# jonasrothfuss/ProMP

Measured on AMD Instinct MI355X. Metric: env-steps/sec through GAE+inner+outer update, higher is better.
Workload: dtype f32

## Files before the change

### include/promp_hip.h

```cpp
#ifndef PROMP_HIP_H
#define PROMP_HIP_H

#include <stddef.h>
#include <stdint.h>

#ifdef __cplusplus
extern "C" {
#endif

typedef struct promp_ctx promp_ctx;

typedef struct promp_dims {
    int32_t n_tasks;
    int32_t n_tasks_global;
    int32_t obs_dim;
    int32_t act_dim;
    int32_t hidden1, hidden2;
    int32_t num_inner_steps;
    int32_t max_rows;
    int32_t max_paths;
    int32_t n_hidden;
    int32_t hidden3, hidden4;
    int32_t hidden_act;
} promp_dims;
// ... 40 lines not shown
int promp_stage_wait(promp_ctx* ctx);
void* promp_host_alloc(size_t bytes);
void promp_host_free(void* p);

int promp_process_samples(promp_ctx* ctx, int step, const promp_proc_opts* opts);

int promp_download_processed(promp_ctx* ctx, int step, float* returns, float* advantages, double* coeffs,
                             double* path_returns0, double* path_undiscounted, double* path_reward_sumsq);

int promp_download_raw(promp_ctx* ctx, int step, double* returns64, double* raw_advantages64);

int promp_set_coeffs(promp_ctx* ctx, int step, int baseline_kind, const double* coeffs);
int promp_predict_baseline(promp_ctx* ctx, int step, int baseline_kind, double* baselines_out);

int promp_set_advantages(promp_ctx* ctx, int step, const float* advantages);
int promp_set_dice_rewards(promp_ctx* ctx, int step, const float* rewards);

int promp_set_theta(promp_ctx* ctx, const float* theta);
int promp_get_theta(promp_ctx* ctx, float* theta);
int promp_set_step_sizes(promp_ctx* ctx, const float* step_sizes);
int promp_set_learn_std(promp_ctx* ctx, int learn_std);
int promp_set_min_std(promp_ctx* ctx, float min_std);
int promp_set_schedule(promp_ctx* ctx, int stage_overlap, int fuse_min_tasks);
int promp_set_primal_cache(promp_ctx* ctx, int on);
int promp_set_reuse_adapt(promp_ctx* ctx, int on);
long long promp_adapt_passes_skipped(promp_ctx* ctx);
long long promp_constraint_hvp_cached_passes(promp_ctx* ctx);
long long promp_state_version(promp_ctx* ctx);
int promp_set_adam_state(promp_ctx* ctx, const float* m, const float* v, int64_t t);
int promp_get_adam_state(promp_ctx* ctx, float* m, float* v, int64_t* t);
int promp_switch_to_pre_update(promp_ctx* ctx);
int promp_set_task_thetas(promp_ctx* ctx, const float* theta_tasks);
int promp_get_task_thetas(promp_ctx* ctx, float* theta_tasks);

int promp_inner_adapt(promp_ctx* ctx, int step, int inner_kind);

int promp_policy_forward(promp_ctx* ctx, const float* obs, int batch, float* mean_out);

int promp_begin_rollout(promp_ctx* ctx, int step, int envs_per_task, int path_length);
int promp_begin_collection(promp_ctx* ctx, int step, int envs_per_task, int max_steps);
int promp_end_collection(promp_ctx* ctx, int step, int n_paths, const int32_t* task_path_offsets, const int32_t* path_env,
                         const int32_t* path_start, const int32_t* path_len, const float* rewards);
int promp_policy_step(promp_ctx* ctx, int step, int t, const float* obs, uint64_t seed, int clip_infos, float* actions_out);
int promp_set_rewards(promp_ctx* ctx, int step, const float* rewards);
int promp_set_rewards_f64(promp_ctx* ctx, int step, const double* rewards);

// ... 51 lines not shown
```

### promp_amd/_lib.py

```python
import ctypes as C
import os

import weakref

import numpy as np

_HERE = os.path.dirname(os.path.abspath(__file__))
DEFAULT_LIBRARY = os.path.join(_HERE, 'libpromp_hip.so')

BASELINE_ZERO, BASELINE_LINEAR_FEATURE, BASELINE_LINEAR_TIME = 0, 1, 2
INNER_RATIO, INNER_LOGLIK, INNER_DICE = 0, 1, 2
OUTER_CLIP, OUTER_RATIO, OUTER_KL, OUTER_LOGLIK = 0, 1, 2, 3
LOSS_RATIO, LOSS_CLIP, LOSS_LOGLIK, LOSS_KL = 0, 1, 2, 3
KERNEL_FWD_BWD, KERNEL_HVP, KERNEL_GRAM, KERNEL_FWD, KERNEL_EXCHANGE = 0, 1, 2, 3, 4


class PrompError(RuntimeError):
    pass


class Dims(C.Structure):
    _fields_ = [('n_tasks', C.c_int32), ('n_tasks_global', C.c_int32), ('obs_dim', C.c_int32), ('act_dim', C.c_int32),
                ('hidden1', C.c_int32), ('hidden2', C.c_int32), ('num_inner_steps', C.c_int32),
                ('max_rows', C.c_int32), ('max_paths', C.c_int32),
# ... 24 lines not shown
    'promp_last_error': (C.c_char_p, []),
    'promp_abi_version': (C.c_int, []),
    'promp_param_count': (C.c_int, [C.POINTER(Dims)]),
    'promp_feature_dim': (C.c_int, [C.POINTER(Dims), C.c_int]),
    'promp_sync': (C.c_int, [_P]),
    'promp_upload_step': (C.c_int, [_P, C.c_int, C.c_int, _I, _I, _F, _F, _F, _F, _F, C.c_int]),
    'promp_process_samples': (C.c_int, [_P, C.c_int, C.POINTER(ProcOpts)]),
    'promp_download_processed': (C.c_int, [_P, C.c_int, _F, _F, _D, _D, _D, _D]),
    'promp_download_raw': (C.c_int, [_P, C.c_int, _D, _D]),
    'promp_set_coeffs': (C.c_int, [_P, C.c_int, C.c_int, _D]),
    'promp_predict_baseline': (C.c_int, [_P, C.c_int, C.c_int, _D]),
    'promp_set_advantages': (C.c_int, [_P, C.c_int, _F]),
    'promp_set_theta': (C.c_int, [_P, _F]),
    'promp_get_theta': (C.c_int, [_P, _F]),
    'promp_set_step_sizes': (C.c_int, [_P, _F]),
    'promp_set_learn_std': (C.c_int, [_P, C.c_int]),
    'promp_set_primal_cache': (C.c_int, [_P, C.c_int]),
    'promp_set_reuse_adapt': (C.c_int, [_P, C.c_int]),
    'promp_adapt_passes_skipped': (C.c_longlong, [_P]),
    'promp_constraint_hvp_cached_passes': (C.c_longlong, [_P]),
    'promp_state_version': (C.c_longlong, [_P]),
    'promp_set_min_std': (C.c_int, [_P, C.c_float]),
    'promp_set_schedule': (C.c_int, [_P, C.c_int, C.c_int]),
    'promp_set_rewards_f64': (C.c_int, [_P, C.c_int, _D]),
    'promp_stage_step': (C.c_int, [_P, C.c_int, C.c_int, _I, _I, _F, _F, _F, _F, _F, C.c_int]),
    'promp_commit_step': (C.c_int, [_P, C.c_int]),
    'promp_stage_wait': (C.c_int, [_P]),
    'promp_host_alloc': (C.c_void_p, [C.c_size_t]),
    'promp_host_free': (None, [C.c_void_p]),
    'promp_constraint_hvp': (C.c_int, [_P, C.c_int, _F, C.c_int, _F]),
    'promp_cg_solve': (C.c_int, [_P, C.c_int, _F, C.c_int, C.c_float, C.c_float, C.c_int, C.c_float, _F, C.POINTER(C.c_double)]),
    'promp_set_adam_state': (C.c_int, [_P, _F, _F, C.c_int64]),
    'promp_get_adam_state': (C.c_int, [_P, _F, _F, C.POINTER(C.c_int64)]),
    'promp_switch_to_pre_update': (C.c_int, [_P]),
    'promp_set_task_thetas': (C.c_int, [_P, _F]),
    'promp_get_task_thetas': (C.c_int, [_P, _F]),
    'promp_inner_adapt': (C.c_int, [_P, C.c_int, C.c_int]),
    'promp_policy_forward': (C.c_int, [_P, _F, C.c_int, _F]),
    'promp_rollout_point_env': (C.c_int, [_P, C.c_int, C.c_int, C.c_int, _D, _D, _F, C.POINTER(PointEnvOpts)]),
    'promp_begin_rollout': (C.c_int, [_P, C.c_int, C.c_int, C.c_int]),
    'promp_begin_collection': (C.c_int, [_P, C.c_int, C.c_int, C.c_int]),
    'promp_end_collection': (C.c_int, [_P, C.c_int, C.c_int, _P, _P, _P, _P, _F]),
    'promp_policy_step': (C.c_int, [_P, C.c_int, C.c_int, _F, C.c_uint64, C.c_int, _F]),
    'promp_set_rewards': (C.c_int, [_P, C.c_int, _F]),
    'promp_download_step': (C.c_int, [_P, C.c_int, _F, _F, _F, _F, _F]),
    'promp_meta_grad': (C.c_int, [_P, C.c_float, _F, C.c_int, C.c_int, _F, _F]),
# ... 590 lines not shown
                   old_mean=np.empty((R, A), np.float32), old_log_std=np.empty((ls_rows, A), np.float32))
        self._call('promp_download_step', int(step), _ptr(out['obs'], C.c_float), _ptr(out['act'], C.c_float),
                   _ptr(out['rew'], C.c_float), _ptr(out['old_mean'], C.c_float), _ptr(out['old_log_std'], C.c_float))
        return out

    def inner_adapt(self, step, inner_kind=INNER_RATIO):
        self._call('promp_inner_adapt', int(step), int(inner_kind))

    def meta_grad(self, clip_eps, inner_kl_coeff, inner_kind=INNER_RATIO, outer_kind=OUTER_CLIP):
        eta = _f32(inner_kl_coeff)
        assert eta.shape == (self.K,)
        grad, stats = np.empty(self.n_params, np.float32), np.empty(self.K + 2, np.float32)
        self._call('promp_meta_grad', float(clip_eps), _ptr(eta, C.c_float), int(inner_kind), int(outer_kind),
                   _ptr(grad, C.c_float), _ptr(stats, C.c_float))
        return grad, dict(loss=float(stats[0]), inner_kl=stats[1:1 + self.K].copy(), outer_kl=float(stats[1 + self.K]))

    def meta_eval(self, clip_eps, inner_kl_coeff, inner_kind=INNER_RATIO, outer_kind=OUTER_CLIP):
        r = self.optimize(0, 0.0, clip_eps, inner_kl_coeff, inner_kind, outer_kind)
        return dict(loss=r['loss_after'], inner_kl=r['inner_kl'], outer_kl=r['outer_kl'])

    def set_schedule(self, stage_overlap=-1, fuse_min_tasks=-1):
        self._call('promp_set_schedule', int(stage_overlap), int(fuse_min_tasks))

    def set_primal_cache(self, on=True):
        self._call('promp_set_primal_cache', -1 if on is None else int(bool(on)))

    def set_reuse_adapt(self, on=True):
        self._call('promp_set_reuse_adapt', int(bool(on)))

    def adapt_passes_skipped(self):
        return int(self.lib.cdll.promp_adapt_passes_skipped(self._h))

    def state_version(self):
        return int(self.lib.cdll.promp_state_version(self._h))

    def constraint_hvp_cached_passes(self):
        return int(self.lib.cdll.promp_constraint_hvp_cached_passes(self._h))

    def set_min_std(self, min_std):
        self._call('promp_set_min_std', float(min_std))

    def set_learn_std(self, on=True):
        self._call('promp_set_learn_std', int(bool(on)))

    def adam_step(self, lr):
        self._call('promp_adam_step', float(lr))
# ... 156 lines not shown
```

### promp_amd/csrc/promp_hip.hip

```cpp
#include "promp_kernels_chain.h"
#include "promp_kernels_pass.h"
#include "promp_kernels_policy.h"
#include "promp_kernels_policy_wide.h"
#include "promp_kernels_wide_bf16.h"
#include "promp_kernels_sample.h"
#include "promp_kernels_rollout.h"
#include "promp_kernels_generic.h"
#include "promp_kernels_generic_bf16.h"
#include "../../include/promp_hip.h"

#include <algorithm>
#include <cmath>
#include <cstdarg>
#include <cstdio>
#include <cstdlib>
#include <cstring>
#include <memory>
#include <string>
#include <vector>

#define PROMP_ARCH_NAME(prop) (prop).gcnArchName

namespace {

// ... 173 lines not shown
    bool tasks_shared = false;
    DevBuf<float> wbuf;
    DevBuf<float> partials, scal_inner, scal_outer, scal_tmp;
    DevBuf<float> red, grad_mean, stats;
    float eta_last[PROMP_ETA_MAX] = {};
    DevBuf<double> gram_partials, red64;
    DevBuf<char> rollout_buf;
    DevBuf<float> stage_rows;
    DevBuf<double> fit_scratch;
    size_t smem_fwd = 0, smem_hvp = 0;
    PassFamily family = PassFamily::Chain;
    int wb_cls = 0;
    size_t smem_wb_fwd = 0, smem_wb_bwd = 0, smem_wb_hvp = 0;
    DevBuf<unsigned> wb_planes, wb_vplanes;
    DevBuf<unsigned> wb_planes_meta;
    DevBuf<float> cg_buf;
    DevBuf<double> cg_scal;
    struct { bool valid = false; unsigned long long theta_version = 0, data_version = 0, sizes_version = 0; const void* step = nullptr; } wbp;
    DevBuf<unsigned> vdir_absmax;
    bool gramt_single = false;
    bool gram_untiled = false;
    int gramt_map_nblk = -1;
    GramtMap gramt_map;
    bool fit_one_launch = false;
    bool gen_bf16 = true;
    DevBuf<unsigned short> gb_wplanes, gb_vplanes;
    long long gb_plane_stride = 0;
    int gb_pf_off[GEN_MAX_LIN] = {}, gb_pb_off[GEN_MAX_LIN] = {};
    int n_lin = 0, g_maxw = 0;
    GenLin lin[GEN_MAX_LIN];
    DevBuf<float> g_act[GEN_MAX_LIN], g_ract[GEN_MAX_LIN], g_mu, g_rmu, g_dz[2], g_qz[2];
    DevBuf<unsigned long long> dbg;
    bool dbg_enabled = false;
    DevBuf<int> task_counters;
    DevBuf<int> split_events;
    ncclComm_t comm = nullptr;
    int rank = 0, nranks = 1;
    float min_log_std = -13.815510558f;
    bool learn_std = true;
    int fuse_min_tasks = 1 << 30;
    int stats_slot = 0;
    int primal_cache = -1;
    unsigned long long version_counter = 0, theta_version = 0, sizes_version = 0;
    unsigned long long cache_counter = 0;
    unsigned long long opt_theta_version = 0;
    struct { bool valid = false; unsigned long long theta_version = 0, data_version = 0, sizes_version = 0; int inner_kind = 0; bool cached = false; float min_log_std = 0.f; bool learn_std = true; } adapt0;
// ... 692 lines not shown
    }
    {
        const int lds = 160 * 1024;
#define PROMP_CHAIN_LDS(N1, N2, KS) if (allow_lds(lds, k_chain_hvp<N1, N2, KS, CHAIN_NW_HVP, false>, k_chain_hvp<N1, N2, KS, CHAIN_NW_HVP, true>)) return -2;
        PROMP_CHAIN_ALL(PROMP_CHAIN_LDS)
#undef PROMP_CHAIN_LDS
#define PROMP_PASS_LDS(N1, N2) \
    if (allow_lds(lds, k_pass<N1, N2, CHAIN_NW_HVP, true, true>, k_pass<N1, N2, CHAIN_NW_HVP, true, false>, k_pass<N1, N2, CHAIN_NW_HVP, false, false>)) return -2;
        PROMP_PASS_ALL(PROMP_PASS_LDS)
#undef PROMP_PASS_LDS
#define PROMP_WB_LDS(CLS, NKO, NXB) if (allow_lds(lds, k_wb_hvp<NKO, NXB>, k_wb_fwd_bwd<NKO, NXB, true>, k_wb_fwd_bwd<NKO, NXB, false>)) return -2;
        PROMP_WB_ALL(PROMP_WB_LDS)
#undef PROMP_WB_LDS
#define PROMP_WIDE_LDS(HH, NOB) if (allow_lds(lds, k_wide_fwd_bwd<HH, NOB, true>, k_wide_fwd_bwd<HH, NOB, false>, k_wide_hvp<HH, NOB>)) return -2;
        PROMP_WIDE_ALL(PROMP_WIDE_LDS)
#undef PROMP_WIDE_LDS
#define PROMP_GEN_LDS(NBW)                                                                                                   \
    if (allow_lds(lds, k_gen_linear<GEN_FWD, NBW>, k_gen_linear<GEN_FWD_T, NBW>, k_gen_linear<GEN_BWD, NBW>, k_gen_linear<GEN_BWD_T, NBW>, \
                  k_gen_wgrad<1, NBW>, k_gen_wgrad<2, NBW>, k_gb_linear<GEN_FWD, NBW>, k_gb_linear<GEN_FWD_T, NBW>,            \
                  k_gb_linear<GEN_BWD, NBW>, k_gb_linear<GEN_BWD_T, NBW>, k_gb_wgrad<1, NBW>, k_gb_wgrad<2, NBW>)) return -2;
        PROMP_GEN_LDS(1) PROMP_GEN_LDS(2) PROMP_GEN_LDS(3) PROMP_GEN_LDS(4)
#undef PROMP_GEN_LDS
        if (allow_lds((int)gen_loss_smem(GEN_MAX_A), k_gen_loss<true, true>, k_gen_loss<false, true>, k_gen_loss<false, false>)) return -2;
#define PROMP_GRAM_INST(NBLK) k_gram<NBLK>,
#define PROMP_FITWV_INST(DT) k_fit_wave<DT>,
        if (allow_lds(lds, PROMP_GRAM_ALL(PROMP_GRAM_INST) PROMP_FITWV_ALL(PROMP_FITWV_INST) k_fit, k_gram_wide, k_gram_tiled<GRAMT_TB, GRAMT_NWV, GRAMT_NLD>, k_fitw_panel<32>, k_fitw_panel<16>,
                      k_fitw_update<32>, k_fitw_update<16>, k_fitw_back<32>, k_fitw_back<16>, k_fit_wide<32>, k_fit_wide<16>)) return -2;
#undef PROMP_GRAM_INST
#undef PROMP_FITWV_INST
    }
    const size_t NP = c->NP, MNP = (size_t)M * NP;
    if (c->theta.alloc(NP) || c->step_sizes.alloc(NP)) return -2;
    if (c->adam_m.alloc(NP) || c->adam_v.alloc(NP)) return -2;
    if (c->theta_tasks.alloc(MNP) || c->chain.alloc((size_t)(K + 1) * MNP)) return -2;
    if (c->lam.alloc(MNP) || c->vbuf.alloc(MNP)) return -2;
    if (c->family == PassFamily::CoopSplit) {
        const size_t pw = (size_t)M * wb_planes_words(wb_nko(c->wb_cls));
        if (c->wb_planes.alloc(pw) || c->wb_vplanes.alloc(pw) || c->wb_planes_meta.alloc(pw)) return -2;
        if (c->vdir_absmax.alloc((size_t)M)) return -2;
    }
    if (c->partials.alloc((size_t)c->max_work * c->partial_stride)) return -2;
    if (c->scal_inner.alloc((size_t)K * M * 2) || c->scal_outer.alloc((size_t)M * 2)) return -2;
    if (c->scal_tmp.alloc((size_t)M * 2)) return -2;
    if (c->red.alloc(NP + K + 2) || c->grad_mean.alloc(NP)) return -2;
    if (c->stats.alloc((size_t)2 * (K + 2))) return -2;
    if (c->red64.alloc(64)) return -2;
    if (c->family == PassFamily::Layered) {
        const size_t R = (size_t)dims->max_rows;
        for (int l = 1; l < c->n_lin; ++l)
// ... 334 lines not shown
    if (o->baseline_kind == PROMP_BASELINE_LINEAR_FEATURE && c->d.obs_dim > PROMP_LINFEAT_MAX_O)
        return fail(-1, "LinearFeatureBaseline's fit is sized for obs_dim <= %d (%d here: %d feature columns); fit LinearTimeBaseline / no "
                    "baseline on the device, or hand advantages in through promp_set_advantages", PROMP_LINFEAT_MAX_O, c->d.obs_dim,
                    2 * c->d.obs_dim + 5);
    SampleArgs a = sample_args(c, S, o->baseline_kind);
    a.work = S.work[0];
    a.task_wg_offsets = S.task_wg_offsets[0];
    a.gamma = o->discount; a.lam = o->gae_lambda; a.reg = o->reg_coeff;
    a.normalize = o->normalize_adv; a.positive = o->positive_adv;
    a.ret64 = S.ret64; a.ret32 = S.ret32; a.adv32 = S.adv32;
    a.path_ret0 = S.path_ret0; a.path_undisc = S.path_undisc; a.path_rsq = S.path_rsq;
    S.feat_dim = a.D;
    const bool on_side = c->overlap && !c->prof && step >= 1;
    hipStream_t st = on_side ? c->side : c->stream;
    if (o->baseline_kind != PROMP_BASELINE_ZERO && fit_buffers(c, on_side)) return -2;
    a.gram_partials = on_side ? c->gram_partials_side : c->gram_partials;
    double* fit_scratch = on_side ? c->fit_scratch_side : c->fit_scratch;
    if (on_side) {
        if (mark_use(c, S)) return -2;
        if (S.use_set) HIPCHECK(hipStreamWaitEvent(c->side, S.ev_use, 0));
        if (S.wait_ready_side) HIPCHECK(hipStreamWaitEvent(c->side, S.ev_ready, 0));
    }
    S.wait_ready_side = false;
    PROMP_LAUNCH(k_returns, dim3(S.n_paths), 64, 0, st, a);
    HIPCHECK(hipGetLastError());
    if (a.kind != BASE_ZERO) {
        const int nblk = (a.D + 1 + 15) / 16;
        if (prof_begin(c, PROMP_KERNEL_GRAM, S.n_rows)) return -2;
        const bool small = nblk <= 5 && (a.O <= 32 || a.kind != BASE_LINFEAT);
        switch (small ? nblk : 0) {
#define PROMP_GRAM_CASE(NBLK) \
    case NBLK: { auto k = k_gram<NBLK>; PROMP_LAUNCH(k, dim3(S.n_work[0]), 64 * GramCfg<NBLK>::NW, GramCfg<NBLK>::SMEM_BYTES, st, a); } break;
            PROMP_GRAM_ALL(PROMP_GRAM_CASE)
#undef PROMP_GRAM_CASE
            default:
                if (nblk >= GRAMT_MIN_NBLK && !c->gram_untiled) {
                    const int nr = gramt_nrect(nblk);
                    int rows, db;
                    gramt_cfg(nblk, a.O, 64 * GRAMT_NWV * GRAMT_NLD, c->gramt_single, &rows, &db);
                    if (c->gramt_map_nblk != nblk) { gramt_balance(nblk, GRAMT_NWV, &c->gramt_map); c->gramt_map_nblk = nblk; }
                    auto k = k_gram_tiled<GRAMT_TB, GRAMT_NWV, GRAMT_NLD>;
                    PROMP_LAUNCH(k, dim3(S.n_work[0], (nr + GRAMT_NWV - 1) / GRAMT_NWV), 64 * GRAMT_NWV, gramt_smem(nblk, rows, db), st, a, nblk,
                                 c->gramt_map, rows, db);
                    break;
                }
                PROMP_LAUNCH(k_gram_wide, dim3(S.n_work[0], gramw_slices(nblk)), 512, gramw_smem(nblk, a.O, gramw_rows(nblk, a.O)), st, a, nblk,
                             gramw_rows(nblk, a.O));
        }
        HIPCHECK(hipGetLastError());
        if (prof_end(c, PROMP_KERNEL_GRAM)) return -2;
        const int DA = a.D + 1;
        if (small) {
            const size_t fit_smem = sizeof(double) * ((size_t)2 * DA * DA + 3 * DA + 2 + fitwv_aux(64));
#define PROMP_FITWV_CASE(DT) else if (DA <= DT) { auto k = k_fit_wave<DT>; PROMP_LAUNCH(k, dim3(c->d.n_tasks), FITWV_NT, fit_smem, st, a, nblk); }
            if (false) {}
            PROMP_FITWV_ALL(PROMP_FITWV_CASE)
            else PROMP_LAUNCH(k_fit, dim3(c->d.n_tasks), 256, fit_smem, st, a, nblk);
#undef PROMP_FITWV_CASE
        } else {
            PROMP_LAUNCH(k_gram_sum_wide, dim3(c->d.n_tasks * fitw_sum_split(nblk)), 256, 0, st, a, nblk, fit_scratch, fitw_sum_split(nblk));
            HIPCHECK(hipGetLastError());
            const int* none = nullptr;
            int* bad = (int*)(fit_scratch + (size_t)c->d.n_tasks * 2 * (c->Dmax + 1) * (c->Dmax + 1));
            const bool phases = a.D >= FITW_ML_MIN_D && !c->fit_one_launch;
#define PROMP_FITW(NB)                                                                                                              \
    if (phases) {                                                                                                                   \
        auto kp = k_fitw_panel<NB>; auto ku = k_fitw_update<NB>; auto kb = k_fitw_back<NB>; auto kf = k_fit_wide<NB>;              \
        for (int k0 = 0; k0 < a.D; k0 += NB) {                                                                                      \
            PROMP_LAUNCH(kp, dim3(c->d.n_tasks), FITW_NT, fitw_panel_smem(a.D, NB), st, a, fit_scratch, k0);                        \
            if (k0 + NB < a.D) PROMP_LAUNCH(ku, dim3(c->d.n_tasks, FITW_UPD_SPLIT), FITW_NT, fitw_panel_smem(a.D, NB), st, a, fit_scratch, k0); \
        }                                                                                                                           \
        PROMP_LAUNCH(kb, dim3(c->d.n_tasks), FITW_NT, fitw_back_smem(a.D, NB), st, a, fit_scratch, bad);                               \
        PROMP_LAUNCH(kf, dim3(c->d.n_tasks), FITW_NT, fitw_smem(a.D, NB), st, a, nblk, fit_scratch, (const int*)bad);               \
    } else { auto k = k_fit_wide<NB>; PROMP_LAUNCH(k, dim3(c->d.n_tasks), FITW_NT, fitw_smem(a.D, NB), st, a, nblk, fit_scratch, none); }
            if (fitw_nb(a.D) == 32) { PROMP_FITW(32) } else { PROMP_FITW(16) }
#undef PROMP_FITW
        }
        HIPCHECK(hipGetLastError());
    }
    PROMP_LAUNCH(k_gae, dim3(S.n_paths), 64, sizeof(double) * (size_t)(a.D > 0 ? a.D : 1), st, a);
    HIPCHECK(hipGetLastError());
    a.work = S.work[1];
    PROMP_LAUNCH(k_normalize, dim3(S.n_work[1]), 256, 0, st, a);
    HIPCHECK(hipGetLastError());
    if (on_side) {
        HIPCHECK(hipEventRecord(S.ev_done, c->side));
        S.side_pending = true;
    }
    S.processed = true;
    S.has_adv = true;
    return 0;
}

int promp_download_processed(promp_ctx* c, int step, float* returns, float* adv, double* coeffs, double* ret0,
                             double* undisc, double* rsq) {
    StepScope sc(c, step, false, false);
    if (sc.rc) return sc.rc;
    StepData& S = sc.S();
    if (!S.processed) return fail(-3, "step %d has not been processed", step);
    hipStream_t st = c->stream;
    if (returns) HIPCHECK(hipMemcpyAsync(returns, S.ret32, sizeof(float) * S.n_rows, hipMemcpyDeviceToHost, st));
    if (adv) HIPCHECK(hipMemcpyAsync(adv, S.adv32, sizeof(float) * S.n_rows, hipMemcpyDeviceToHost, st));
    const size_t P = (size_t)S.n_paths, NC = (coeffs && S.feat_dim > 0) ? (size_t)c->d.n_tasks * c->coeff_stride : 0;
    if (c->small_host.reserve(3 * P + NC, 1)) return -2;
    double* h = c->small_host;
    if (ret0) HIPCHECK(hipMemcpyAsync(h, S.path_ret0, sizeof(double) * P, hipMemcpyDeviceToHost, st));
    if (undisc) HIPCHECK(hipMemcpyAsync(h + P, S.path_undisc, sizeof(double) * P, hipMemcpyDeviceToHost, st));
// ... 137 lines not shown
}
int promp_set_step_sizes(promp_ctx* c, const float* s) {
    NEED_CTX(c);
    c->sizes_version = ++c->version_counter;
    if (params_in(c, c->step_sizes, s, 1)) return -2;
    return mask_log_std_step_sizes(c);
}
int promp_set_min_std(promp_ctx* c, float min_std) {
    NEED_CTX(c);
    if (!(min_std > 0.f)) return fail(-1, "min_std must be positive");
    c->min_log_std = logf(min_std);
    c->version_counter += 1;
    return 0;
}
int promp_set_schedule(promp_ctx* c, int stage_overlap, int fuse_min_tasks) {
    NEED_CTX(c);
    if (stage_overlap >= 0) {
        HIPCHECK(hipStreamSynchronize(c->side));
        c->overlap = stage_overlap != 0;
    }
    if (fuse_min_tasks >= 0) c->fuse_min_tasks = fuse_min_tasks;
    return 0;
}
int promp_set_reuse_adapt(promp_ctx* c, int on) {
    NEED_CTX(c);
    c->reuse_adapt = on != 0;
    c->adapt0.valid = false;
    return 0;
}
long long promp_adapt_passes_skipped(promp_ctx* c) { return c ? c->adapt_passes_skipped : -1; }
long long promp_constraint_hvp_cached_passes(promp_ctx* c) { return c ? c->chvp_cached_passes : -1; }
long long promp_state_version(promp_ctx* c) { return c ? (long long)c->version_counter : -1; }
int promp_set_primal_cache(promp_ctx* c, int on) {
    NEED_CTX(c);
    c->primal_cache = on < 0 ? -1 : on != 0;
    return 0;
}
int promp_set_learn_std(promp_ctx* c, int on) {
    NEED_CTX(c);
    if (on && !c->learn_std) return fail(-3, "learn_std cannot be switched back on: the log_std step sizes were zeroed (set the step sizes again)");
    c->learn_std = on != 0;
    c->sizes_version = ++c->version_counter;
    return mask_log_std_step_sizes(c);
}
static int tasks_materialize(promp_ctx* c);
int promp_set_task_thetas(promp_ctx* c, const float* t) {
// ... 755 lines not shown
```

### promp_amd/csrc/promp_kernels_sample.h

```cpp
#pragma once
#include <utility>
#include "promp_device.h"
#include "promp_kernels_policy.h"

enum { BASE_ZERO = 0, BASE_LINFEAT = 1, BASE_LINTIME = 2 };

struct SampleArgs {
    const float* obs;
    const float* rew;
    const double* rew64;
    const int* path_row_offsets;
    const int* path_task;
    const int* row_t;
    const int* task_row_offsets;
    const int* task_path_offsets;
    const WorkItem* work;
    const int* task_wg_offsets;
    int O, D, kind;
    double gamma, lam, reg;
    int normalize, positive;
    double* ret64;
    float* ret32;
    double* adv64;
    float* adv32;
// ... 70 lines not shown
        for (int end = T; end > 0; end -= 64) {
            const int t = end - 64 + lane;
            const double x = (t >= 0) ? (double)a.c[row0 + t] : 0.0;
            const double y = dice_suffix_chunk(x, lane) + carry;
            if (t >= 0) a.tmp[row0 + t] = y;
            carry = shfl_idx_f64(y, 0);
        }
        total = carry;
    }
    double carry = 0.0;
    for (int end = T; end > 0; end -= 64) {
        const int t = end - 64 + lane;
        double x = 0.0;
        if (t >= 0) {
            x = (double)a.rw[row0 + t];
            if (a.mode == 1) x *= total - a.tmp[row0 + t] + (double)a.c[row0 + t];
        }
        const double y = dice_suffix_chunk(x, lane) + carry;
        if (t >= 0) a.out[row0 + t] = (float)y;
        carry = shfl_idx_f64(y, 0);
    }
}

template <int NBLK>
struct GramCfg {
    static constexpr int NW = (NBLK <= 3) ? 8 : 4;
    static constexpr int FS = (NBLK % 2 == 1) ? 16 * NBLK : 16 * NBLK + 16;
    static constexpr int NPAIR = NBLK * (NBLK + 1) / 2;
    static constexpr int WAVE_BYTES = 16 * FS * 8 + 16 * 32 * 4 + 2 * 16 * 8;
    static constexpr int SLAB_BYTES = NW * NPAIR * 256 * 8;
    static constexpr int SMEM_BYTES = (NW * WAVE_BYTES > SLAB_BYTES) ? NW * WAVE_BYTES : SLAB_BYTES;
};

#ifdef PROMP_DEV_STAMPS
#define SA_STAMPS unsigned long long ph[8] = {0, 0, 0, 0, 0, 0, 0, 0}, tph = promp_clock()
#define SA_PHASE(i) do { const unsigned long long now_ = promp_clock(); ph[i] += now_ - tph; tph = now_; } while (0)
#else
#define SA_STAMPS do { } while (0)
#define SA_PHASE(i) do { } while (0)
#endif
template <int NBLK>
__global__ void __launch_bounds__(64 * GramCfg<NBLK>::NW) k_gram(SampleArgs a) {
    SA_STAMPS;
    constexpr int NW = GramCfg<NBLK>::NW, FS = GramCfg<NBLK>::FS, NPAIR = GramCfg<NBLK>::NPAIR, NC = 16 * NBLK;
    PROMP_SMEM_DECL;
    unsigned char* smem = (unsigned char*)PROMP_SMEM_PTR;
    const int tid = threadIdx.x, lane = tid & 63, w = tid >> 6, i16 = lane & 15, kk = lane >> 4;
    double* Phi = (double*)(smem + (size_t)w * GramCfg<NBLK>::WAVE_BYTES);
    const WorkItem wk = a.work[blockIdx.x];
    const int O = a.O, D = a.D;
    f64x4 acc[NPAIR];
#pragma unroll
    for (int p = 0; p < NPAIR; ++p) acc[p] = zero4d();
    float xr[8];
    double tr = 0.0;
    int ttr = 0;
    auto request = [&](int base) {
        const bool live = base < wk.row_end;
        const int nrows = !live ? 0 : (wk.row_end - base) < 16 ? (wk.row_end - base) : 16;
        const long long b0 = live ? base : wk.row_begin;
        if (a.kind == BASE_LINFEAT) {
            const int lim = nrows * O;
#pragma unroll
            for (int u = 0; u < 8; ++u) {
                const int e = lane + 64 * u;
                const float x = a.obs[b0 * O + (e < lim ? e : 0)];
                xr[u] = (e < lim) ? x : 0.f;
            }
        }
        if (lane < 16) {
            const int r = lane < nrows ? lane : 0;
            tr = a.ret64[b0 + r];
            ttr = a.row_t[b0 + r];
        }
    };
    int poff[8];
#pragma unroll
    for (int u = 0; u < 8; ++u) {
        const int e = lane + 64 * u, r = e / (O > 0 ? O : 1);
        poff[u] = (a.kind == BASE_LINFEAT && e < 16 * O) ? r * FS + (e - r * O) : -1;
    }
    for (int e = lane; e < 16 * FS; e += 64) Phi[e] = 0.0;
    wave_sync();
    const int qt = (a.kind == BASE_LINFEAT) ? 2 * O : 0;
    request(wk.row_begin + 16 * w);
    SA_PHASE(0);
    for (int base = wk.row_begin + 16 * w; base < wk.row_end; base += 16 * NW) {
        const int nrows = (wk.row_end - base) < 16 ? (wk.row_end - base) : 16;
#pragma unroll
        for (int u = 0; u < 8; ++u)
            if (poff[u] >= 0) {
                const float oc = fminf(fmaxf(xr[u], -10.f), 10.f);
                Phi[poff[u]] = (double)oc;
                Phi[poff[u] + O] = (double)(oc * oc);
            }
        if (lane < 16) {
            const bool rv = lane < nrows;
            const double tau = rv ? (double)ttr / 100.0 : 0.0;
            double* pr = Phi + lane * FS;
            pr[qt] = tau;
            pr[qt + 1] = tau * tau;
            pr[qt + 2] = tau * tau * tau;
            pr[qt + 3] = rv ? 1.0 : 0.0;
            pr[D] = rv ? tr : 0.0;
        }
        SA_PHASE(1);
// ... 131 lines not shown
        const int k0 = J + 2 + 8 * b;
        double m[8];
        sched_fence();
#pragma unroll
        for (int u = 0; u < 8; ++u) m[u] = (k0 + u < DT) ? readlane_f64(W[J], k0 + u) : 0.0;
#pragma unroll
        for (int u = 0; u < 8; ++u)
            if (k0 + u < DT) W[k0 + u] -= W[J] * m[u];
        sched_fence();
        if (b == 0) e = rsq_e(dn, r0);
        if (b == 1 || (b == 0 && NBATCH == 1)) rs = rsq_finish(r0, e);
    }
    if (NBATCH <= 0) rs = rsq_finish(r0, rsq_e(dn, r0));
}
template <int DT, int... Js>
PROMP_DEV void fitw_columns(double (&W)[DT], double* colbuf, double* rsv, int lane, int D, std::integer_sequence<int, Js...>) {
    const double d0 = readlane_f64(W[0], 0), s0 = rsq_seed(d0);
    double rs = rsq_finish(s0, rsq_e(d0, s0));
    (fitw_column<Js, DT>(W, colbuf, rsv, rs, lane, D), ...);
}

#define FITWV_NT 512
template <int DT>
__global__ void __launch_bounds__(FITWV_NT) k_fit_wave(SampleArgs a, int NBLK) {
    PROMP_SMEM_DECL;
    SA_STAMPS;
    const int D = a.D, DA = D + 1;
    double* colbuf = (double*)PROMP_SMEM_PTR;
    double* rsv = colbuf + DT * FITWV_CS + 2;
    double* G = colbuf + fitwv_aux(DT);
    const int lane = threadIdx.x & 63, task = blockIdx.x;
    const int NPAIR = NBLK * (NBLK + 1) / 2;
    const int wg0 = a.task_wg_offsets[task], wg1 = a.task_wg_offsets[task + 1];
    {
        constexpr int NE = 5;
        double sacc[NE];
#pragma unroll
        for (int q = 0; q < NE; ++q) sacc[q] = 0.0;
        for (int base = wg0; base < wg1; base += 16) {
            double v[NE][16];
#pragma unroll
            for (int q = 0; q < NE; ++q) {
                const int e = threadIdx.x + q * FITWV_NT;
                if (e < NPAIR * 256) {
#pragma unroll
                    for (int u = 0; u < 16; ++u) {
                        const int wg = base + u < wg1 ? base + u : wg1 - 1;
                        v[q][u] = a.gram_partials[(long long)wg * (NPAIR * 256) + e];
                    }
                }
            }
#pragma unroll
            for (int q = 0; q < NE; ++q) {
                const int e = threadIdx.x + q * FITWV_NT;
// ... 35 lines not shown
        SA_PHASE(1);
        wave_fence();
        double y = (lane < D) ? colbuf[lane * FITWV_CS + D] : 0.0;
        const double rdg = rsv[lane < D ? lane : 0];
#pragma unroll
        for (int k = 0; k < DT; ++k) {
            const double l = colbuf[row * FITWV_CS + (k < DA ? k : 0)];
            W[k] = (k < D && row < k) ? l : 0.0;
        }
        SA_PHASE(2);
#pragma unroll
        for (int j = DT - 1; j >= 0; --j) {
            if (j < D) {
                const double wj = readlane_f64(y * rdg, j);
                y -= W[j] * wj;
            }
        }
        wsol = y * rdg;
        wave_sync();
        SA_PHASE(3);
        if (!wave_any(lane < D && wsol != wsol)) break;
        reg *= 10.0;
    }
    if (lane < D) a.coeffs[(long long)task * a.coeff_stride + lane] = wsol;
#ifdef PROMP_DEV_STAMPS
    if (task == 0 && lane == 0)
        printf("k_fit_wave cycles: partial sums %llu | factorisation %llu | column reads %llu | back substitution %llu\n", ph[0], ph[1], ph[2], ph[3]);
#endif
}

__global__ void __launch_bounds__(64) k_gae(SampleArgs a) {
    PROMP_SMEM_DECL;
    double* wc = (double*)PROMP_SMEM_PTR;
    const int p = blockIdx.x, lane = threadIdx.x;
    const int row0 = a.path_row_offsets[p], T = a.path_row_offsets[p + 1] - row0;
    const int task = a.path_task[p];
    const int O = a.O, D = a.D;
    if (a.kind != BASE_ZERO)
        for (int i = lane; i < D; i += 64) wc[i] = a.coeffs[(long long)task * a.coeff_stride + i];
    __syncthreads();
    const double g = a.gamma, gl = a.gamma * a.lam;
    const double f = pow(gl, (double)(64 - lane));
    double carry = 0.0, bcarry = 0.0, s1 = 0.0, s2 = 0.0, mn = 1e300;
    for (int end = T; end > 0; end -= 64) {
        const int t = end - 64 + lane;
        const bool valid = t >= 0;
        const long long row = (long long)row0 + t;
        double b = 0.0;
        if (valid && a.kind != BASE_ZERO) {
            int q = 0;
// ... 787 lines not shown
```

Before: 291.6 million.

## Fuse returns into Gram kernel and fit+GAE+normalize into one per-task launch

Adds a stage-A mode, on by default, that computes discounted returns inside the Gram kernel. The separate fit, GAE and normalization kernels become a single per-task kernel that fits the baseline, predicts it, runs the GAE scan and normalizes advantages. This cuts the stage from four or five launches to two and removes the inter-kernel round trips. The cost is less parallelism: GAE runs one block per task instead of one per path. Returns are also recomputed across work-item boundaries, and the cross-block visibility of returns inside the Gram launch depends on relaxed atomic loads and barriers.

```diff
diff --git a/include/promp_hip.h b/include/promp_hip.h
--- a/include/promp_hip.h
+++ b/include/promp_hip.h
@@ -86,6 +86,8 @@
 int promp_set_learn_std(promp_ctx* ctx, int learn_std);
 int promp_set_min_std(promp_ctx* ctx, float min_std);
 int promp_set_schedule(promp_ctx* ctx, int stage_overlap, int fuse_min_tasks);
+int promp_set_stage_a(promp_ctx* ctx, int mode);
+int promp_stage_a_launches(promp_ctx* ctx);
 int promp_set_primal_cache(promp_ctx* ctx, int on);
 int promp_set_reuse_adapt(promp_ctx* ctx, int on);
 long long promp_adapt_passes_skipped(promp_ctx* ctx);
diff --git a/promp_amd/_lib.py b/promp_amd/_lib.py
--- a/promp_amd/_lib.py
+++ b/promp_amd/_lib.py
@@ -70,6 +70,8 @@
     'promp_state_version': (C.c_longlong, [_P]),
     'promp_set_min_std': (C.c_int, [_P, C.c_float]),
     'promp_set_schedule': (C.c_int, [_P, C.c_int, C.c_int]),
+    'promp_set_stage_a': (C.c_int, [_P, C.c_int]),
+    'promp_stage_a_launches': (C.c_int, [_P]),
     'promp_set_rewards_f64': (C.c_int, [_P, C.c_int, _D]),
     'promp_stage_step': (C.c_int, [_P, C.c_int, C.c_int, _I, _I, _F, _F, _F, _F, _F, C.c_int]),
     'promp_commit_step': (C.c_int, [_P, C.c_int]),
@@ -706,6 +708,12 @@
     def set_schedule(self, stage_overlap=-1, fuse_min_tasks=-1):
         self._call('promp_set_schedule', int(stage_overlap), int(fuse_min_tasks))
 
+    def set_stage_a(self, mode=1):
+        self._call('promp_set_stage_a', int(mode))
+
+    def stage_a_launches(self):
+        return int(self.lib.cdll.promp_stage_a_launches(self._h))
+
     def set_primal_cache(self, on=True):
         self._call('promp_set_primal_cache', -1 if on is None else int(bool(on)))
 
diff --git a/promp_amd/csrc/promp_hip.hip b/promp_amd/csrc/promp_hip.hip
--- a/promp_amd/csrc/promp_hip.hip
+++ b/promp_amd/csrc/promp_hip.hip
@@ -219,6 +219,8 @@
     bool gram_untiled = false;
     int gramt_map_nblk = -1;
     GramtMap gramt_map;
+    int stage_a_mode = 1;
+    int stage_a_launches = 0;
     bool fit_one_launch = false;
     bool gen_bf16 = true;
     DevBuf<unsigned short> gb_wplanes, gb_vplanes;
@@ -957,9 +959,9 @@
         PROMP_GEN_LDS(1) PROMP_GEN_LDS(2) PROMP_GEN_LDS(3) PROMP_GEN_LDS(4)
 #undef PROMP_GEN_LDS
         if (allow_lds((int)gen_loss_smem(GEN_MAX_A), k_gen_loss<true, true>, k_gen_loss<false, true>, k_gen_loss<false, false>)) return -2;
-#define PROMP_GRAM_INST(NBLK) k_gram<NBLK>,
-#define PROMP_FITWV_INST(DT) k_fit_wave<DT>,
-        if (allow_lds(lds, PROMP_GRAM_ALL(PROMP_GRAM_INST) PROMP_FITWV_ALL(PROMP_FITWV_INST) k_fit, k_gram_wide, k_gram_tiled<GRAMT_TB, GRAMT_NWV, GRAMT_NLD>, k_fitw_panel<32>, k_fitw_panel<16>,
+#define PROMP_GRAM_INST(NBLK) k_gram<NBLK, false>, k_gram<NBLK, true>,
+#define PROMP_FITWV_INST(DT) k_fit_wave<DT>, k_fit_gae<DT>,
+        if (allow_lds(lds, PROMP_GRAM_ALL(PROMP_GRAM_INST) PROMP_FITWV_ALL(PROMP_FITWV_INST) k_fit_gae<0>, k_fit, k_gram_wide, k_gram_tiled<GRAMT_TB, GRAMT_NWV, GRAMT_NLD>, k_fitw_panel<32>, k_fitw_panel<16>,
                       k_fitw_update<32>, k_fitw_update<16>, k_fitw_back<32>, k_fitw_back<16>, k_fit_wide<32>, k_fit_wide<16>)) return -2;
 #undef PROMP_GRAM_INST
 #undef PROMP_FITWV_INST
@@ -1340,15 +1342,23 @@
         if (S.wait_ready_side) HIPCHECK(hipStreamWaitEvent(c->side, S.ev_ready, 0));
     }
     S.wait_ready_side = false;
-    PROMP_LAUNCH(k_returns, dim3(S.n_paths), 64, 0, st, a);
-    HIPCHECK(hipGetLastError());
+    const int nblk = (a.D + 1 + 15) / 16;
+    const bool small = nblk <= 5 && (a.O <= 32 || a.kind != BASE_LINFEAT);
+    const bool fused = c->stage_a_mode != 0 && small;
+    int launches = 0;
+    if (!fused || a.kind == BASE_ZERO) {
+        PROMP_LAUNCH(k_returns, dim3(S.n_paths), 64, 0, st, a);
+        HIPCHECK(hipGetLastError());
+        ++launches;
+    }
     if (a.kind != BASE_ZERO) {
-        const int nblk = (a.D + 1 + 15) / 16;
         if (prof_begin(c, PROMP_KERNEL_GRAM, S.n_rows)) return -2;
-        const bool small = nblk <= 5 && (a.O <= 32 || a.kind != BASE_LINFEAT);
         switch (small ? nblk : 0) {
-#define PROMP_GRAM_CASE(NBLK) \
-    case NBLK: { auto k = k_gram<NBLK>; PROMP_LAUNCH(k, dim3(S.n_work[0]), 64 * GramCfg<NBLK>::NW, GramCfg<NBLK>::SMEM_BYTES, st, a); } break;
+#define PROMP_GRAM_CASE(NBLK)                                                                                                              \
+    case NBLK:                                                                                                                             \
+        if (fused) { auto k = k_gram<NBLK, true>; PROMP_LAUNCH(k, dim3(S.n_work[0]), 64 * GramCfg<NBLK>::NW, GramCfg<NBLK>::SMEM_BYTES, st, a); }  \
+        else { auto k = k_gram<NBLK, false>; PROMP_LAUNCH(k, dim3(S.n_work[0]), 64 * GramCfg<NBLK>::NW, GramCfg<NBLK>::SMEM_BYTES, st, a); }       \
+        break;
             PROMP_GRAM_ALL(PROMP_GRAM_CASE)
 #undef PROMP_GRAM_CASE
             default:
@@ -1366,18 +1376,22 @@
                              gramw_rows(nblk, a.O));
         }
         HIPCHECK(hipGetLastError());
+        ++launches;
         if (prof_end(c, PROMP_KERNEL_GRAM)) return -2;
         const int DA = a.D + 1;
-        if (small) {
+        if (fused && DA <= 64) {
+        } else if (small) {
             const size_t fit_smem = sizeof(double) * ((size_t)2 * DA * DA + 3 * DA + 2 + fitwv_aux(64));
 #define PROMP_FITWV_CASE(DT) else if (DA <= DT) { auto k = k_fit_wave<DT>; PROMP_LAUNCH(k, dim3(c->d.n_tasks), FITWV_NT, fit_smem, st, a, nblk); }
             if (false) {}
             PROMP_FITWV_ALL(PROMP_FITWV_CASE)
             else PROMP_LAUNCH(k_fit, dim3(c->d.n_tasks), 256, fit_smem, st, a, nblk);
 #undef PROMP_FITWV_CASE
+            ++launches;
         } else {
             PROMP_LAUNCH(k_gram_sum_wide, dim3(c->d.n_tasks * fitw_sum_split(nblk)), 256, 0, st, a, nblk, fit_scratch, fitw_sum_split(nblk));
             HIPCHECK(hipGetLastError());
+            launches += 2;
             const int* none = nullptr;
             int* bad = (int*)(fit_scratch + (size_t)c->d.n_tasks * 2 * (c->Dmax + 1) * (c->Dmax + 1));
             const bool phases = a.D >= FITW_ML_MIN_D && !c->fit_one_launch;
@@ -1396,11 +1410,24 @@
         }
         HIPCHECK(hipGetLastError());
     }
-    PROMP_LAUNCH(k_gae, dim3(S.n_paths), 64, sizeof(double) * (size_t)(a.D > 0 ? a.D : 1), st, a);
-    HIPCHECK(hipGetLastError());
-    a.work = S.work[1];
-    PROMP_LAUNCH(k_normalize, dim3(S.n_work[1]), 256, 0, st, a);
-    HIPCHECK(hipGetLastError());
+    if (fused) {
+        const int DA = a.D + 1;
+        const size_t sm = fitgae_smem(a.D, a.kind == BASE_LINFEAT ? a.O : 0);
+#define PROMP_FITGAE_CASE(DT) else if (DA <= DT) { auto k = k_fit_gae<DT>; PROMP_LAUNCH(k, dim3(c->d.n_tasks), FITWV_NT, sm, st, a, nblk); }
+        if (a.kind == BASE_ZERO || DA > 64) { auto k = k_fit_gae<0>; PROMP_LAUNCH(k, dim3(c->d.n_tasks), FITWV_NT, sm, st, a, nblk); }
+        PROMP_FITWV_ALL(PROMP_FITGAE_CASE)
+#undef PROMP_FITGAE_CASE
+        HIPCHECK(hipGetLastError());
+        ++launches;
+    } else {
+        PROMP_LAUNCH(k_gae, dim3(S.n_paths), 64, sizeof(double) * (size_t)(a.D > 0 ? a.D : 1), st, a);
+        HIPCHECK(hipGetLastError());
+        a.work = S.work[1];
+        PROMP_LAUNCH(k_normalize, dim3(S.n_work[1]), 256, 0, st, a);
+        HIPCHECK(hipGetLastError());
+        launches += 2;
+    }
+    c->stage_a_launches = launches;
     if (on_side) {
         HIPCHECK(hipEventRecord(S.ev_done, c->side));
         S.side_pending = true;
@@ -1584,6 +1611,13 @@
     if (fuse_min_tasks >= 0) c->fuse_min_tasks = fuse_min_tasks;
     return 0;
 }
+int promp_set_stage_a(promp_ctx* c, int mode) {
+    NEED_CTX(c);
+    if (mode < 0 || mode > 1) return fail(-1, "stage-A mode %d (0: one launch per stage, 1: returns in the Gram launch and one launch per task)", mode);
+    c->stage_a_mode = mode;
+    return 0;
+}
+int promp_stage_a_launches(promp_ctx* c) { return c ? c->stage_a_launches : -1; }
 int promp_set_reuse_adapt(promp_ctx* c, int on) {
     NEED_CTX(c);
     c->reuse_adapt = on != 0;
diff --git a/promp_amd/csrc/promp_kernels_sample.h b/promp_amd/csrc/promp_kernels_sample.h
--- a/promp_amd/csrc/promp_kernels_sample.h
+++ b/promp_amd/csrc/promp_kernels_sample.h
@@ -116,6 +116,61 @@
     }
 }
 
+#ifdef PROMP_EMU
+PROMP_DEV double load_f64_l2(const double* p) { return *p; }
+#else
+PROMP_DEV double load_f64_l2(const double* p) { return __hip_atomic_load(p, __ATOMIC_RELAXED, __HIP_MEMORY_SCOPE_AGENT); }
+#endif
+
+PROMP_DEV void returns_of_item(const SampleArgs& a, const WorkItem& wk, int w, int NW, int lane) {
+    const int p0 = a.task_path_offsets[wk.task], p1 = a.task_path_offsets[wk.task + 1];
+    const bool last_item = wk.row_end == a.task_row_offsets[wk.task + 1];
+    int lo = p0, hi = p1 - 1;
+    while (lo < hi) {
+        const int mid = (lo + hi) >> 1;
+        if (a.path_row_offsets[mid + 1] > wk.row_begin) hi = mid; else lo = mid + 1;
+    }
+    while (lo > p0 && a.path_row_offsets[lo - 1] >= wk.row_begin) --lo;
+    const double g = a.gamma;
+    const double f = pow(g, (double)(64 - lane));
+    for (int p = lo + w; p < p1; p += NW) {
+        const int row0 = a.path_row_offsets[p], T = a.path_row_offsets[p + 1] - row0;
+        if (row0 > wk.row_end || (row0 == wk.row_end && !last_item)) break;
+        const bool own = row0 >= wk.row_begin;
+        double carry = 0.0, usum = 0.0, rsq = 0.0, y0 = 0.0;
+        for (int end = T; end > 0; end -= 64) {
+            if (row0 + end <= wk.row_begin) break;
+            const int t = end - 64 + lane;
+            const int rr = row0 + (t >= 0 ? t : 0);
+            const double x = (t >= 0) ? (a.rew64 ? a.rew64[rr] : (double)a.rew[rr]) : 0.0;
+            double y = x, gg = g;
+#pragma unroll
+            for (int d = 1; d < 64; d <<= 1) {
+                const double up = shfl_down_f64(y, d);
+                if (lane + d < 64) y += gg * up;
+                gg *= gg;
+            }
+            y += f * carry;
+            if (t >= 0 && rr >= wk.row_begin && rr < wk.row_end) {
+                a.ret64[rr] = y;
+                a.ret32[rr] = (float)y;
+            }
+            if (t == 0) y0 = y;
+            carry = shfl_idx_f64(y, 0);
+            usum += x;
+            rsq += x * x;
+        }
+        usum = wave_sum_f64(usum);
+        rsq = wave_sum_f64(rsq);
+        y0 = wave_sum_f64(y0);
+        if (own && lane == 0) {
+            a.path_ret0[p] = y0;
+            a.path_undisc[p] = usum;
+            a.path_rsq[p] = rsq;
+        }
+    }
+}
+
 template <int NBLK>
 struct GramCfg {
     static constexpr int NW = (NBLK <= 3) ? 8 : 4;
@@ -133,7 +188,7 @@
 #define SA_STAMPS do { } while (0)
 #define SA_PHASE(i) do { } while (0)
 #endif
-template <int NBLK>
+template <int NBLK, bool RET>
 __global__ void __launch_bounds__(64 * GramCfg<NBLK>::NW) k_gram(SampleArgs a) {
     SA_STAMPS;
     constexpr int NW = GramCfg<NBLK>::NW, FS = GramCfg<NBLK>::FS, NPAIR = GramCfg<NBLK>::NPAIR, NC = 16 * NBLK;
@@ -164,7 +219,7 @@
         }
         if (lane < 16) {
             const int r = lane < nrows ? lane : 0;
-            tr = a.ret64[b0 + r];
+            tr = RET ? load_f64_l2(a.ret64 + b0 + r) : a.ret64[b0 + r];
             ttr = a.row_t[b0 + r];
         }
     };
@@ -176,6 +231,10 @@
     }
     for (int e = lane; e < 16 * FS; e += 64) Phi[e] = 0.0;
     wave_sync();
+    if (RET) {
+        returns_of_item(a, wk, w, NW, lane);
+        __syncthreads();
+    }
     const int qt = (a.kind == BASE_LINFEAT) ? 2 * O : 0;
     request(wk.row_begin + 16 * w);
     SA_PHASE(0);
@@ -353,14 +412,12 @@
 
 #define FITWV_NT 512
 template <int DT>
-__global__ void __launch_bounds__(FITWV_NT) k_fit_wave(SampleArgs a, int NBLK) {
-    PROMP_SMEM_DECL;
+PROMP_DEV void fit_wave_task(const SampleArgs& a, int NBLK, double* colbuf, int task, double* wout, const char* who) {
     SA_STAMPS;
     const int D = a.D, DA = D + 1;
-    double* colbuf = (double*)PROMP_SMEM_PTR;
     double* rsv = colbuf + DT * FITWV_CS + 2;
     double* G = colbuf + fitwv_aux(DT);
-    const int lane = threadIdx.x & 63, task = blockIdx.x;
+    const int lane = threadIdx.x & 63;
     const int NPAIR = NBLK * (NBLK + 1) / 2;
     const int wg0 = a.task_wg_offsets[task], wg1 = a.task_wg_offsets[task + 1];
     {
@@ -442,10 +499,184 @@
         if (!wave_any(lane < D && wsol != wsol)) break;
         reg *= 10.0;
     }
-    if (lane < D) a.coeffs[(long long)task * a.coeff_stride + lane] = wsol;
+    if (lane < D) {
+        a.coeffs[(long long)task * a.coeff_stride + lane] = wsol;
+        if (wout != nullptr) wout[lane] = wsol;
+    }
 #ifdef PROMP_DEV_STAMPS
     if (task == 0 && lane == 0)
-        printf("k_fit_wave cycles: partial sums %llu | factorisation %llu | column reads %llu | back substitution %llu\n", ph[0], ph[1], ph[2], ph[3]);
+        printf("%s cycles: partial sums %llu | factorisation %llu | column reads %llu | back substitution %llu\n", who, ph[0], ph[1], ph[2], ph[3]);
+#else
+    (void)who;
+#endif
+}
+template <int DT>
+__global__ void __launch_bounds__(FITWV_NT) k_fit_wave(SampleArgs a, int NBLK) {
+    PROMP_SMEM_DECL;
+    fit_wave_task<DT>(a, NBLK, (double*)PROMP_SMEM_PTR, blockIdx.x, nullptr, "k_fit_wave");
+}
+
+#define FITGAE_HEAD 80
+PROMP_HD size_t fitgae_smem(int D, int O) {
+    const size_t DA = (size_t)D + 1, fit = sizeof(double) * (DA * DA + fitwv_aux(64)), tile = sizeof(float) * FITWV_NT * (size_t)(O | 1);
+    return sizeof(double) * FITGAE_HEAD + (fit > tile ? fit : tile);
+}
+template <int DT>
+__global__ void __launch_bounds__(FITWV_NT) k_fit_gae(SampleArgs a, int NBLK) {
+    PROMP_SMEM_DECL;
+    SA_STAMPS;
+    constexpr int NT = FITWV_NT, NW = FITWV_NT / 64;
+    double* wc = (double*)PROMP_SMEM_PTR;
+    double* st = wc + FITGAE_HEAD - 4;
+    double* body = wc + FITGAE_HEAD;
+    const int tid = threadIdx.x, lane = tid & 63, w = tid >> 6, task = blockIdx.x;
+    const int O = a.O, D = a.D;
+    if (a.kind != BASE_ZERO) {
+        if constexpr (DT > 0) fit_wave_task<DT>(a, NBLK, body, task, wc, "k_fit_gae: fit");
+        else
+            for (int i = tid; i < D; i += NT) wc[i] = a.coeffs[(long long)task * a.coeff_stride + i];
+    }
+    __syncthreads();
+    SA_PHASE(0);
+    const int rb = a.task_row_offsets[task], re = a.task_row_offsets[task + 1];
+    if (a.kind != BASE_ZERO) {
+        float* tile = (float*)body;
+        const int OS = O | 1, q = (a.kind == BASE_LINFEAT) ? 2 * O : 0;
+        const int dr = NT / (O > 0 ? O : 1), dc = NT - dr * O;
+        for (int base = rb; base < re; base += NT) {
+            const int nr = (re - base) < NT ? (re - base) : NT;
+            if (a.kind == BASE_LINFEAT) {
+                const int lim = nr * O;
+                const float* src = a.obs + (long long)base * O;
+                float x[32];
+#pragma unroll
+                for (int u = 0; u < 32; ++u) {
+                    const int e = tid + u * NT;
+                    x[u] = (e < lim) ? src[e] : 0.f;
+                }
+                int r = tid / (O > 0 ? O : 1), c = tid - r * O;
+#pragma unroll
+                for (int u = 0; u < 32; ++u) {
+                    if (tid + u * NT < lim) tile[r * OS + c] = x[u];
+                    r += dr;
+                    c += dc;
+                    if (c >= O) { c -= O; ++r; }
+                }
+                __syncthreads();
+            }
+            if (tid < nr) {
+                const long long row = (long long)base + tid;
+                double b = 0.0;
+                if (a.kind == BASE_LINFEAT)
+                    for (int c = 0; c < O; ++c) {
+                        const float o = tile[tid * OS + c];
+                        const float oc = fminf(fmaxf(o, -10.f), 10.f);
+                        b += wc[c] * (double)oc + wc[O + c] * (double)(oc * oc);
+                    }
+                const double tau = (double)a.row_t[row] / 100.0;
+                b += wc[q] * tau + wc[q + 1] * (tau * tau) + wc[q + 2] * (tau * tau * tau) + wc[q + 3];
+                a.adv64[row] = b;
+                if (a.bl64 != nullptr) a.bl64[row] = b;
+            }
+            __syncthreads();
+        }
+    }
+    SA_PHASE(1);
+    {
+        const double g = a.gamma, gl = a.gamma * a.lam;
+        const double f = pow(gl, (double)(64 - lane));
+        const bool fitted = a.kind != BASE_ZERO;
+        for (int p = a.task_path_offsets[task] + w; p < a.task_path_offsets[task + 1]; p += NW) {
+            const int row0 = a.path_row_offsets[p], T = a.path_row_offsets[p + 1] - row0;
+            double carry = 0.0, bcarry = 0.0, s1 = 0.0, s2 = 0.0, mn = 1e300;
+            double bq = 0.0, rq = 0.0;
+            auto request = [&](int end) {
+                const int t = end - 64 + lane;
+                const long long rr = (long long)row0 + ((end > 0 && t >= 0) ? t : 0);
+                rq = (T > 0) ? (a.rew64 ? a.rew64[rr] : (double)a.rew[rr]) : 0.0;
+                bq = (fitted && T > 0) ? load_f64_l2(a.adv64 + rr) : 0.0;
+            };
+            request(T);
+            for (int end = T; end > 0; end -= 64) {
+                const int t = end - 64 + lane;
+                const bool valid = t >= 0;
+                const long long row = (long long)row0 + t;
+                const double b = valid ? bq : 0.0, rw = rq;
+                request(end - 64);
+                double bn = shfl_down_f64(b, 1);
+                if (lane == 63) bn = bcarry;
+                const double x = valid ? (rw + g * bn - b) : 0.0;
+                double y = x, gg = gl;
+#pragma unroll
+                for (int d = 1; d < 64; d <<= 1) {
+                    const double up = shfl_down_f64(y, d);
+                    if (lane + d < 64) y += gg * up;
+                    gg *= gg;
+                }
+                y += f * carry;
+                if (valid) {
+                    a.adv64[row] = y;
+                    s1 += y;
+                    s2 += y * y;
+                    mn = y < mn ? y : mn;
+                }
+                carry = shfl_idx_f64(y, 0);
+                bcarry = shfl_idx_f64(b, 0);
+            }
+            s1 = wave_sum_f64(s1);
+            s2 = wave_sum_f64(s2);
+            mn = wave_min_f64(mn);
+            if (lane == 0) {
+                a.path_mom[3 * p + 0] = s1;
+                a.path_mom[3 * p + 1] = s2;
+                a.path_mom[3 * p + 2] = mn;
+            }
+        }
+    }
+    __syncthreads();
+    SA_PHASE(2);
+    if (tid == 0) {
+        double s1 = 0.0, s2 = 0.0, mn = 1e300;
+        for (int p = a.task_path_offsets[task]; p < a.task_path_offsets[task + 1]; ++p) {
+            const double m0 = load_f64_l2(a.path_mom + 3 * p), m1 = load_f64_l2(a.path_mom + 3 * p + 1), m2 = load_f64_l2(a.path_mom + 3 * p + 2);
+            s1 += m0;
+            s2 += m1;
+            mn = m2 < mn ? m2 : mn;
+        }
+        const double n = (double)(re - rb);
+        const double mean = s1 / n;
+        double var = s2 / n - mean * mean;
+        var = var > 0.0 ? var : 0.0;
+        st[0] = mean;
+        st[1] = sqrt(var);
+        st[2] = mn;
+    }
+    __syncthreads();
+    {
+        const double mean = st[0], sd = st[1];
+        double mn = st[2];
+        if (a.normalize) mn = (mn - mean) / (sd + 1e-8);
+        for (int base = rb + tid; base < re; base += 8 * NT) {
+            double x[8];
+#pragma unroll
+            for (int u = 0; u < 8; ++u) {
+                const int row = base + u * NT;
+                x[u] = load_f64_l2(a.adv64 + (row < re ? row : base));
+            }
+#pragma unroll
+            for (int u = 0; u < 8; ++u) {
+                const int row = base + u * NT;
+                double v = x[u];
+                if (a.normalize) v = (v - mean) / (sd + 1e-8);
+                if (a.positive) v = (v - mn) + 1e-8;
+                if (row < re) a.adv32[row] = (float)v;
+            }
+        }
+    }
+    SA_PHASE(3);
+#ifdef PROMP_DEV_STAMPS
+    if (task == 0 && tid == 0)
+        printf("k_fit_gae cycles (thread 0 of task 0): fit %llu | predictions %llu | GAE %llu | normalisation %llu\n", ph[0], ph[1], ph[2], ph[3]);
 #endif
 }
 
```

Result: slower. 286.8 million (-1.6%).
